# ZenGo-X/multi-party-ecdsa

Measured on AMD Instinct MI355X. Metric: GG20 signatures/sec (t=1, n=3; all parties of each session on the node's GPUs) + Paillier-2048 modexp/s per GPU, higher is better.
Workload: dtype u32 limbs (radix 2^29) / u64 accumulators

## Files before the change

### multi_party_ecdsa_amd/csrc/mpe_internal.h

```cpp
#pragma once
#include <hip/hip_runtime.h>
#include <stdint.h>
#include <new>
#include <utility>
#include <string>
#include <vector>

#include "../../include/mpecdsa_hip.h"
#include "mpe_kernels_heavy.h"
#include "mpe_sched.h"

struct mpe_ctx {
  int device = 0;
  int cus = 256;
  int fb_window_bits = 13;
  int window_bits = 0;
  bool ec_lane_groups = true;
  bool adaptive_lanes = true;
  bool use_pown = true;
  bool use_pair = true;
  bool use_multiexp = true;
  bool use_crt = true;
  bool use_fixed_base = true;
  bool use_sliding = true;
  int wide_div = 4;
  int device_share = 1;
  int xwide_div = 16;
  bool merge_xn = true;
  int use_prio = 1;
  int ladder_prio = 1;
  int use_crt_n = 1;
  int no_pdl_ahead = 0;
  int no_r1_dlog_first = 0;
  int no_r1_inversion_ahead = 0;
  int merge_r1_quarters = 1;
  bool merge_r1 = true;
  size_t fb_budget_bytes = 0;
  int modexp_waves_per_cu = 8;
  int fb_split = 0;
  int gg20_trace = 0;
  int sampler_max_attempts = 128;
  int no_primaries = 0;
  int no_elect = 0;
  int grid_mode = 2;
  void* tables[6] = {nullptr, nullptr, nullptr, nullptr, nullptr, nullptr};
  size_t tables_bytes[6] = {0, 0, 0, 0, 0, 0};
  hipStream_t aux[3] = {nullptr, nullptr, nullptr};
  hipEvent_t ev_fork[2] = {nullptr, nullptr}, ev_join[3] = {nullptr, nullptr, nullptr};
  hipEvent_t ev_ahead = nullptr;
  hipEvent_t ev_mid = nullptr;
  bool aux_ready = false;
  bool allow_par = true;
  int par_items = 32768;
  void* ws = nullptr;
  size_t ws_bytes = 0, ws_off = 0;
  int ws_hold = 0;
  size_t ws_top = 0;
  void* sess_buf = nullptr;
  size_t sess_bytes = 0;
  bool sess_in_use = false;
  void* slab_buf = nullptr;
  size_t slab_bytes = 0;
  mpe_launch_info last = {};
  mpe_encoding enc = {};
  bool prof_on = false;
  struct ProfEvt { hipEvent_t a, b; int kind, bits, exp_words, batch, exp2_words; int wave_trips; };
  std::vector<ProfEvt> prof;
  uint32_t* prof_ctr = nullptr;
  int prof_ctr_cap = 0;
};

struct mpe_modset {
  int bits = 0;
  int count = 0;
  int K = 0;
  void* blob = nullptr;
  uint32_t* n_limbs = nullptr;
  uint32_t* one_limbs = nullptr;
  uint32_t* r2_limbs = nullptr;
  uint32_t* r2h_limbs = nullptr;
  uint32_t* n0inv = nullptr;
  uint32_t* words = nullptr;
  uint32_t* one_words = nullptr;
};

struct mpe_pairset {
  int half_bits = 0;
  int count = 0;
  void* blob = nullptr;
  uint32_t *n_limbs = nullptr, *n0inv = nullptr, *one = nullptr, *r2 = nullptr, *tp = nullptr, *kc = nullptr;
  const uint32_t* mod_words = nullptr;
};

void mpe_set_error(const char* what, hipError_t e);
void mpe_set_error_msg(const char* what);

namespace mpe {

inline Rows rows(const uint32_t* p, int stride, const int32_t* idx = nullptr, int words = 0) {
  return Rows{p, idx, stride, words};
}
inline Rows no_rows() { return Rows{nullptr, nullptr, 0, 0}; }

int launch_modexp(mpe_ctx* ctx, const mpe_modset* ms, int batch, Rows mod_sel, Rows base_lo, Rows base_hi, Rows exps,
                  int exp_words, uint32_t* out, hipStream_t st);
int launch_modexp2(mpe_ctx* ctx, const mpe_modset* ms, int batch, Rows mod_sel, Rows base, Rows exps, int exp_words,
                   Rows base2, Rows exps2, int exp2_words, uint32_t* out, hipStream_t st);
int launch_modmul(mpe_ctx* ctx, const mpe_modset* ms, int batch, Rows mod_sel, Rows a, Rows b, uint32_t* out,
                  hipStream_t st);
int modset_create_dev(mpe_ctx* ctx, int bits, int count, const uint32_t* d_moduli, mpe_modset** out, hipStream_t st);

void ctx_copy_options(mpe_ctx* dst, const mpe_ctx* src);
void prof_begin(mpe_ctx* ctx, hipStream_t st, int kind, int bits, int exp_words, int batch, int exp2_words = 0);
void prof_end(mpe_ctx* ctx, hipStream_t st);
uint32_t* prof_counter(mpe_ctx* ctx, int wave_trips);

int pairset_create_2048(int count, const uint32_t* d_moduli, mpe_pairset** out, hipStream_t st);
int pairset_create_1024(int count, const uint32_t* d_moduli, mpe_pairset** out, hipStream_t st);
int pair_modexp_2048(mpe_ctx* ctx, const mpe_pairset* ps, int batch, Rows mod_sel, Rows base, Rows exps, int exp_words,
                     Rows base2, Rows exps2, int exp2_words, int half, uint32_t* out, hipStream_t st, int public_exp);
int pair_modexp_1024(mpe_ctx* ctx, const mpe_pairset* ps, int batch, Rows mod_sel, Rows base, Rows exps, int exp_words,
                     Rows base2, Rows exps2, int exp2_words, int half, uint32_t* out, hipStream_t st, int public_exp);

int ws_reserve(mpe_ctx* ctx, size_t bytes, hipStream_t st);
void* ws_alloc(mpe_ctx* ctx, size_t bytes);
uint32_t* tables_for(mpe_ctx* ctx, size_t need, hipStream_t st);
bool ensure_aux(mpe_ctx* ctx);

struct Fork {
  mpe_ctx* ctx; hipStream_t main; int n, first; bool on;
  Fork(mpe_ctx* c, hipStream_t m, int branches, bool enable, int first_aux = 0);
  hipStream_t s(int i) const { return (on && i > 0) ? ctx->aux[first + i - 1] : main; }
  void join();
  void branch_done_wait(int i, hipStream_t waiter);
};
struct WsTop {
  mpe_ctx* c;
  WsTop(mpe_ctx* ctx, const char* top) : c(ctx) { c->ws_top = (size_t)(((const char*)c->ws + c->ws_bytes) - top); }
  ~WsTop() { c->ws_top = 0; }
};
template <class T>
inline T* ws_array(mpe_ctx* ctx, size_t count) { return (T*)ws_alloc(ctx, count * sizeof(T)); }

inline int blocks_for(int n, int threads) { return (n + threads - 1) / threads; }

inline int persistent_grid(const mpe_ctx* ctx, int need, int cap);
inline int ladder_grid(const mpe_ctx* ctx, int units, int cap) {
  if (ctx->no_elect) return persistent_grid(ctx, units, cap);
  if (units <= cap) return (2 * units <= cap && !ctx->no_primaries) ? 2 * units : units;
  return cap;
}
inline SchedArgs ladder_sched(const mpe_ctx* ctx, int units, int cap, int32_t* state, hipStream_t st) {
  SchedArgs a{nullptr, SCHED_STATIC, units, ctx->use_prio ? ctx->ladder_prio : 0};
  if (ctx->no_elect || !state) return a;
  if (2 * units <= cap) { if (!ctx->no_primaries) { a.state = state; a.mode = SCHED_PRIMARIES; } }
  else if (units > cap) { a.state = state; a.mode = SCHED_ALL; }
  if (a.state) (void)hipMemsetAsync(a.state, 0, SCHED_WORDS * sizeof(int32_t), st);
  return a;
}
inline int persistent_grid(const mpe_ctx* ctx, int need, int cap) {
  if (need <= cap) return need;
  const int rem = need % cap;
  if (rem == 0) return cap;
  if (ctx->grid_mode == 1 || (ctx->grid_mode == 2 && 2 * rem <= cap)) return cap;
  const int trips = (need + cap - 1) / cap;
  return (need + trips - 1) / trips;
}

}
```

### multi_party_ecdsa_amd/csrc/mpe_lib.hip

```cpp
#include <string.h>
#include <initializer_list>
#include <mutex>
#include "mpe_internal.h"
#include "mpe_ec.h"

using namespace mpe;

thread_local std::string g_last_error;
void mpe_set_error(const char* what, hipError_t e) { g_last_error = std::string(what) + ": " + hipGetErrorString(e); }
void mpe_set_error_msg(const char* what) { g_last_error = what; }

namespace mpe {

int ws_reserve(mpe_ctx* ctx, size_t bytes, hipStream_t st) {
  if (ctx->ws_hold) {
    if (ctx->ws_off + bytes + ctx->ws_top > ctx->ws_bytes) { mpe_set_error_msg("workspace: the shared reservation is too small"); return MPE_E_NOMEM; }
    return MPE_OK;
  }
  ctx->ws_off = 0;
  if (bytes + ctx->ws_top <= ctx->ws_bytes) return MPE_OK;
  if (ctx->ws_top) { mpe_set_error_msg("workspace: cannot grow while a caller keeps arrays at its top"); return MPE_E_NOMEM; }
  if (ctx->ws) { (void)hipStreamSynchronize(st); (void)hipFree(ctx->ws); ctx->ws = nullptr; ctx->ws_bytes = 0; }
  const size_t want = bytes + (bytes >> 2) + (1u << 20);
  hipError_t e = hipMalloc(&ctx->ws, want);
// ... 1 lines not shown
  ctx->ws_bytes = want;
  return MPE_OK;
}
void* ws_alloc(mpe_ctx* ctx, size_t bytes) {
  const size_t off = (ctx->ws_off + 255) & ~(size_t)255;
  if (off + bytes + ctx->ws_top > ctx->ws_bytes) return nullptr;
  ctx->ws_off = off + bytes;
  return (char*)ctx->ws + off;
}

static int slot_of(const mpe_ctx* ctx, hipStream_t st) {
  for (int i = 0; i < 3; ++i) if (ctx->aux[i] && st == ctx->aux[i]) return i + 1;
  return 0;
}
uint32_t* tables_for(mpe_ctx* ctx, size_t need, hipStream_t st) {
  const int sl = slot_of(ctx, st);
  if (need > ctx->tables_bytes[sl]) {
    if (ctx->tables[sl]) { (void)hipStreamSynchronize(st); (void)hipFree(ctx->tables[sl]); ctx->tables[sl] = nullptr; ctx->tables_bytes[sl] = 0; }
    hipError_t e = hipMalloc(&ctx->tables[sl], need);
    if (e != hipSuccess) { mpe_set_error("hipMalloc(window tables)", e); return nullptr; }
    ctx->tables_bytes[sl] = need;
  }
  return (uint32_t*)ctx->tables[sl];
}
bool ensure_aux(mpe_ctx* ctx) {
  if (ctx->aux_ready) return true;
  for (int i = 0; i < 3; ++i) if (hipStreamCreateWithFlags(&ctx->aux[i], hipStreamNonBlocking) != hipSuccess) return false;
  for (int i = 0; i < 2; ++i) if (hipEventCreateWithFlags(&ctx->ev_fork[i], hipEventDisableTiming) != hipSuccess) return false;
  for (int i = 0; i < 3; ++i) if (hipEventCreateWithFlags(&ctx->ev_join[i], hipEventDisableTiming) != hipSuccess) return false;
  if (hipEventCreateWithFlags(&ctx->ev_mid, hipEventDisableTiming) != hipSuccess) return false;
  if (hipEventCreateWithFlags(&ctx->ev_ahead, hipEventDisableTiming) != hipSuccess) return false;
  ctx->aux_ready = true;
  return true;
}
Fork::Fork(mpe_ctx* c, hipStream_t m, int branches, bool enable, int first_aux) : ctx(c), main(m), n(branches), first(first_aux) {
  on = enable && c->allow_par && branches > 1 && first_aux + branches - 1 <= 3 && ensure_aux(c);
  if (!on) return;
  hipEvent_t ev = c->ev_fork[first_aux ? 1 : 0];
  (void)hipEventRecord(ev, m);
  for (int i = 1; i < n; ++i) (void)hipStreamWaitEvent(c->aux[first + i - 1], ev, 0);
}
void Fork::branch_done_wait(int i, hipStream_t waiter) {
  if (!on || i <= 0 || waiter == ctx->aux[first + i - 1]) return;
  (void)hipEventRecord(ctx->ev_join[first + i - 1], ctx->aux[first + i - 1]);
  (void)hipStreamWaitEvent(waiter, ctx->ev_join[first + i - 1], 0);
}
void Fork::join() {
  if (!on) return;
  for (int i = 1; i < n; ++i) {
    (void)hipEventRecord(ctx->ev_join[first + i - 1], ctx->aux[first + i - 1]);
    (void)hipStreamWaitEvent(main, ctx->ev_join[first + i - 1], 0);
  }
}

void prof_begin(mpe_ctx* ctx, hipStream_t st, int kind, int bits, int exp_words, int batch, int exp2_words) {
  if (!ctx->prof_on) return;
  mpe_ctx::ProfEvt ev;
  ev.kind = kind; ev.bits = bits; ev.exp_words = exp_words; ev.batch = batch; ev.exp2_words = exp2_words; ev.wave_trips = 0;
  (void)hipEventCreate(&ev.a);
  (void)hipEventCreate(&ev.b);
  (void)hipEventRecord(ev.a, st);
  ctx->prof.push_back(ev);
}
uint32_t* prof_counter(mpe_ctx* ctx, int wave_trips) {
  if (!ctx->prof_on || ctx->prof.empty() || !ctx->prof_ctr || (int)ctx->prof.size() > ctx->prof_ctr_cap) return nullptr;
  ctx->prof.back().wave_trips = wave_trips;
  return ctx->prof_ctr + (ctx->prof.size() - 1);
}
void prof_end(mpe_ctx* ctx, hipStream_t st) {
  if (ctx->prof_on && !ctx->prof.empty()) (void)hipEventRecord(ctx->prof.back().b, st);
}

static ModsetView view_of(const mpe_modset* ms) {
  ModsetView v;
  v.n_limbs = ms->n_limbs; v.one_limbs = ms->one_limbs; v.r2_limbs = ms->r2_limbs; v.r2h_limbs = ms->r2h_limbs;
  v.n0inv = ms->n0inv; v.count = ms->count;
  return v;
}

template <class C>
static int grid_for(const mpe_ctx* ctx, int batch, int waves_per_cu) {
  return persistent_grid(ctx, (batch + C::GROUPS - 1) / C::GROUPS, ctx->cus * waves_per_cu);
}

template <class C>
static int modset_create_impl(int count, const uint32_t* d_moduli, mpe_modset** out, hipStream_t st) {
  mpe_modset* ms = new (std::nothrow) mpe_modset();
  if (!ms) return MPE_E_NOMEM;
  ms->bits = C::BITS;
  ms->count = count;
  ms->K = C::K;
  const size_t words = (size_t)count * C::K;
  const size_t iw = (size_t)count * C::K32;
  const size_t total = (4 * words + (size_t)count + iw + 4) * sizeof(uint32_t);
  hipError_t e = hipMalloc(&ms->blob, total);
  if (e != hipSuccess) { delete ms; mpe_set_error("hipMalloc(modset)", e); return MPE_E_NOMEM; }
  uint32_t* p = (uint32_t*)ms->blob;
  ms->n_limbs = p;
  ms->one_limbs = p + words;
  ms->r2_limbs = p + 2 * words;
  ms->r2h_limbs = p + 3 * words;
  ms->n0inv = p + 4 * words;
  ms->words = ms->n0inv + count;
  ms->one_words = ms->words + iw;
  (void)hipMemcpyAsync(ms->words, d_moduli, iw * sizeof(uint32_t), hipMemcpyDeviceToDevice, st);
  (void)hipMemsetD32Async((hipDeviceptr_t)ms->one_words, 1, 1, st);
  const int blocks = (count + C::GROUPS - 1) / C::GROUPS;
  hipLaunchKernelGGL(modset_setup_kernel<C>, dim3(blocks), dim3(64), 0, st, count, d_moduli, ms->n_limbs,
                     ms->one_limbs, ms->r2_limbs, ms->r2h_limbs, ms->n0inv);
  e = hipGetLastError();
  if (e != hipSuccess) { (void)hipFree(ms->blob); delete ms; mpe_set_error("modset_setup_kernel", e); return MPE_E_HIP; }
  *out = ms;
  return MPE_OK;
}

int modset_create_dev(mpe_ctx* ctx, int bits, int count, const uint32_t* d_moduli, mpe_modset** out, hipStream_t st) {
  (void)ctx;
  if (bits == 4096) return modset_create_impl<Cfg4096>(count, d_moduli, out, st);
  if (bits == 2048) return modset_create_impl<Cfg2048>(count, d_moduli, out, st);
  return MPE_E_ARG;
}

template <class C>
static int modexp_impl(mpe_ctx* ctx, const mpe_modset* ms, int batch, Rows mod_sel, Rows base_lo, Rows base_hi, Rows exps,
                       int exp_words, Rows base2, Rows exps2, int exp2_words, uint32_t* d_out, hipStream_t st) {
  const int units = (batch + C::GROUPS - 1) / C::GROUPS, cap = ctx->cus * ctx->modexp_waves_per_cu;
  const int grid = ladder_grid(ctx, units, cap);
  int wb = exp_words <= 8 ? 4 : (exp_words < 48 ? 5 : 6);
  if (ctx->window_bits) wb = ctx->window_bits;
  const bool dual = base2.p != nullptr;
  if (dual && (base_hi.p != nullptr || exp2_words <= 0 || 32 * exp2_words > ((exp_words * 32 + wb - 1) / wb - 1) * wb)) {
    mpe_set_error_msg("modexp: the second exponent must be shorter than the first");
    return MPE_E_ARG;
  }
  const size_t need = (size_t)grid * C::GROUPS * (((size_t)1 << wb) + (dual ? 16 : 0)) * C::K * sizeof(uint32_t);
  uint32_t* tabs = tables_for(ctx, need + SCHED_WORDS * sizeof(int32_t), st);
  if (!tabs) return MPE_E_NOMEM;
  const SchedArgs sched = ladder_sched(ctx, units, cap, (int32_t*)((char*)tabs + need), st);
  prof_begin(ctx, st, 0, C::BITS, exp_words, batch, dual ? exp2_words : 0);
  hipLaunchKernelGGL(modexp_kernel<C>, dim3(grid), dim3(64), 0, st, batch, view_of(ms), mod_sel, base_lo, base_hi, exps,
                     exp_words, wb, base2, exps2, exp2_words, d_out, tabs, sched);
  prof_end(ctx, st);
  hipError_t e = hipGetLastError();
  if (e != hipSuccess) { mpe_set_error("modexp_kernel", e); return MPE_E_HIP; }
  ctx->last.waves = grid;
  ctx->last.ints_per_wave = C::GROUPS;
  ctx->last.limbs = C::K;
  ctx->last.limb_bits = C::W;
  ctx->last.lds_bytes_per_wave = C::LDS_WORDS * 4;
  ctx->last.table_scratch_bytes = need;
  return MPE_OK;
}

int launch_modexp2(mpe_ctx* ctx, const mpe_modset* ms, int batch, Rows mod_sel, Rows base, Rows exps, int exp_words,
                   Rows base2, Rows exps2, int exp2_words, uint32_t* out, hipStream_t st) {
  if (batch == 0) return MPE_OK;
  if (ms->bits == 4096)
    return modexp_impl<Cfg4096>(ctx, ms, batch, mod_sel, base, no_rows(), exps, exp_words, base2, exps2, exp2_words, out, st);
  if (ms->bits == 2048)
    return modexp_impl<Cfg2048>(ctx, ms, batch, mod_sel, base, no_rows(), exps, exp_words, base2, exps2, exp2_words, out, st);
  return MPE_E_ARG;
}
int launch_modexp(mpe_ctx* ctx, const mpe_modset* ms, int batch, Rows mod_sel, Rows base_lo, Rows base_hi, Rows exps,
                  int exp_words, uint32_t* out, hipStream_t st) {
  if (batch == 0) return MPE_OK;
  if (ms->bits == 4096)
    return modexp_impl<Cfg4096>(ctx, ms, batch, mod_sel, base_lo, base_hi, exps, exp_words, no_rows(), no_rows(), 0, out, st);
  if (ms->bits == 2048)
    return modexp_impl<Cfg2048>(ctx, ms, batch, mod_sel, base_lo, base_hi, exps, exp_words, no_rows(), no_rows(), 0, out, st);
  return MPE_E_ARG;
}

template <class C>
static int modmul_impl(mpe_ctx* ctx, const mpe_modset* ms, int batch, Rows mod_sel, Rows a, Rows b, uint32_t* d_out,
                       hipStream_t st) {
  const int grid = grid_for<C>(ctx, batch, 16);
  prof_begin(ctx, st, 1, C::BITS, 0, batch);
  hipLaunchKernelGGL(modmul_kernel<C>, dim3(grid), dim3(64), 0, st, batch, view_of(ms), mod_sel, a, b, d_out);
  prof_end(ctx, st);
  hipError_t e = hipGetLastError();
  if (e != hipSuccess) { mpe_set_error("modmul_kernel", e); return MPE_E_HIP; }
  return MPE_OK;
}

int launch_modmul(mpe_ctx* ctx, const mpe_modset* ms, int batch, Rows mod_sel, Rows a, Rows b, uint32_t* out,
                  hipStream_t st) {
  if (batch == 0) return MPE_OK;
  if (ms->bits == 4096) return modmul_impl<Cfg4096>(ctx, ms, batch, mod_sel, a, b, out, st);
  if (ms->bits == 2048) return modmul_impl<Cfg2048>(ctx, ms, batch, mod_sel, a, b, out, st);
  return MPE_E_ARG;
}

static Rows mod_selector(const mpe_modset* ms, const int32_t* d_mod_idx) {
  return Rows{nullptr, d_mod_idx, (d_mod_idx == nullptr && ms->count != 1) ? 1 : 0, 0};
}

}

#include "mpe_small.h"

namespace mpe {
static void pairset_free(mpe_pairset* ps) {
  if (!ps) return;
  if (ps->blob) (void)hipFree(ps->blob);
  delete ps;
}
static int pairset_create(int half_bits, int count, const uint32_t* d_moduli, mpe_pairset** out, hipStream_t st) {
  if (half_bits == 2048) return pairset_create_2048(count, d_moduli, out, st);
  if (half_bits == 1024) return pairset_create_1024(count, d_moduli, out, st);
  return MPE_E_ARG;
}
static int launch_pair_modexp(mpe_ctx* ctx, const mpe_pairset* ps, int batch, Rows mod_sel, Rows base, Rows exps, int exp_words,
                              Rows base2, Rows exps2, int exp2_words, uint32_t* out, hipStream_t st, int half = 0, int public_exp = 0) {
  if (batch == 0) return MPE_OK;
  if (ps->half_bits == 2048)
    return pair_modexp_2048(ctx, ps, batch, mod_sel, base, exps, exp_words, base2, exps2, exp2_words, half, out, st, public_exp);
  if (ps->half_bits == 1024)
    return pair_modexp_1024(ctx, ps, batch, mod_sel, base, exps, exp_words, base2, exps2, exp2_words, half, out, st, public_exp);
  return MPE_E_ARG;
}
}
#include "mpe_paillier.h"
#include "mpe_proofs.h"
#include "mpe_mta.h"
#include "mpe_bob.h"
#include "mpe_gg20.h"
#include "mpe_sample.h"
#include "mpe_pipeline.h"
#include "mpe_comm.h"
#include "mpe_sigma.h"
#include "mpe_blame.h"
#include "mpe_keygen.h"
#include "mpe_primes.h"
#include "mpe_lindell.h"

extern "C" {

const char* mpe_version(void) { return "mpecdsa-hip 0.7.0 (gfx950)"; }
const char* mpe_last_error(void) { return g_last_error.c_str(); }

void mpe_encoding_default(mpe_encoding* e) {
  if (!e) return;
  memset(e, 0, sizeof *e);
  e->ck_salt = 0x4B5A656Eu;
  for (int i = 0; i < 4; ++i) e->ord_dlog[i] = e->ord_cdlog[i] = (uint8_t)i;
  for (int i = 0; i < 8; ++i) e->ord_pedersen[i] = e->ord_heg[i] = e->ord_ecddh[i] = (uint8_t)i;
}
static bool is_perm(const uint8_t* o, int n) {
  unsigned seen = 0;
  for (int i = 0; i < n; ++i) { if (o[i] >= n || (seen >> o[i]) & 1u) return false; seen |= 1u << o[i]; }
  return true;
}
int mpe_ctx_set_encoding(mpe_ctx* ctx, const mpe_encoding* e) {
  if (!ctx || !e) return MPE_E_ARG;
  if (e->chain_point > 1 || e->zero_bytes > 1 || e->ck_mask_order > 1 || e->reserved != 0 || !is_perm(e->ord_dlog, 3) ||
      !is_perm(e->ord_pedersen, 5) || !is_perm(e->ord_heg, 7) || !is_perm(e->ord_ecddh, 6) || !is_perm(e->ord_cdlog, 4)) {
    mpe_set_error_msg("mpe_ctx_set_encoding: a flag is not 0/1 or an order is not a permutation");
    return MPE_E_ARG;
  }
  ctx->enc = *e;
  return MPE_OK;
}
int mpe_ctx_set_device_share(mpe_ctx* ctx, int contexts) {
  if (!ctx || contexts < 1 || contexts > 64) return MPE_E_ARG;
  ctx->device_share = contexts;
  return MPE_OK;
}
int mpe_ctx_get_encoding(const mpe_ctx* ctx, mpe_encoding* out) {
  if (!ctx || !out) return MPE_E_ARG;
  *out = ctx->enc;
  return MPE_OK;
}

namespace mpe {
struct CtxOption {
  const char* key;
  long lo, hi;
  void (*set)(mpe_ctx*, long);
  long (*get)(const mpe_ctx*);
};
#define MPE_OPT_BOOL_OFF(name, field) {name, 0, 1, [](mpe_ctx* c, long v) { c->field = !v; }, [](const mpe_ctx* c) -> long { return c->field ? 0 : 1; }}
#define MPE_OPT_INT(name, lo, hi, field) {name, lo, hi, [](mpe_ctx* c, long v) { c->field = (decltype(c->field))v; }, [](const mpe_ctx* c) -> long { return (long)c->field; }}
static const CtxOption kCtxOptions[] = {
    MPE_OPT_BOOL_OFF("no_fixed_base", use_fixed_base),
    MPE_OPT_BOOL_OFF("no_crt", use_crt),
    MPE_OPT_BOOL_OFF("no_multiexp", use_multiexp),
    MPE_OPT_BOOL_OFF("no_pair", use_pair),
    MPE_OPT_BOOL_OFF("no_pown", use_pown),
    MPE_OPT_BOOL_OFF("no_sliding", use_sliding),
    MPE_OPT_BOOL_OFF("no_par", allow_par),
    MPE_OPT_BOOL_OFF("no_wide", adaptive_lanes),
    MPE_OPT_BOOL_OFF("no_ec_lane_groups", ec_lane_groups),
    MPE_OPT_BOOL_OFF("no_merge_xn", merge_xn),
    MPE_OPT_BOOL_OFF("no_merge_r1", merge_r1),
    MPE_OPT_INT("fb_window_bits", 4, 16, fb_window_bits),
    MPE_OPT_INT("window_bits", 0, 6, window_bits),
    MPE_OPT_INT("wide_div", 1, 64, wide_div),
    MPE_OPT_INT("merge_r1_quarters", 0, 64, merge_r1_quarters),
    MPE_OPT_INT("no_r1_inversion_ahead", 0, 1, no_r1_inversion_ahead),
    MPE_OPT_BOOL_OFF("no_prio", use_prio),
    MPE_OPT_INT("no_pdl_ahead", 0, 1, no_pdl_ahead),
    MPE_OPT_BOOL_OFF("no_crt_n", use_crt_n),
    MPE_OPT_INT("no_r1_dlog_first", 0, 1, no_r1_dlog_first),
    MPE_OPT_INT("xwide_div", 0, 1 << 20, xwide_div),
    MPE_OPT_INT("waves_per_cu", 1, 8, modexp_waves_per_cu),
    MPE_OPT_INT("grid_mode", 0, 2, grid_mode),
    MPE_OPT_INT("fb_split", 0, 64, fb_split),
    MPE_OPT_INT("gg20_trace", 0, 1, gg20_trace),
    MPE_OPT_INT("sampler_max_attempts", 1, 1 << 20, sampler_max_attempts),
    MPE_OPT_INT("no_primaries", 0, 1, no_primaries),
    MPE_OPT_INT("no_elect", 0, 1, no_elect),
    {"fb_budget_mb", 0, 1 << 20, [](mpe_ctx* c, long v) { c->fb_budget_bytes = (size_t)v << 20; }, [](const mpe_ctx* c) -> long { return (long)(c->fb_budget_bytes >> 20); }},
};
#undef MPE_OPT_BOOL_OFF
#undef MPE_OPT_INT
extern "C++" void ctx_copy_options(mpe_ctx* dst, const mpe_ctx* src) {
  for (const CtxOption& o : kCtxOptions) o.set(dst, o.get(src));
}
}

int mpe_ctx_set_option(mpe_ctx* ctx, const char* key, const char* value) {
  if (!ctx || !key || !value) return MPE_E_ARG;
  if (!strcmp(key, "grid")) {
    const int m = !strcmp(value, "equal") ? 0 : (!strcmp(value, "full") ? 1 : (!strcmp(value, "hybrid") ? 2 : -1));
    if (m < 0) { mpe_set_error_msg("mpe_ctx_set_option: grid = equal | full | hybrid"); return MPE_E_ARG; }
    ctx->grid_mode = m;
    return MPE_OK;
  }
  if (!strcmp(key, "no_adaptive_lanes")) {
    const bool off = atoi(value) != 0;
    ctx->adaptive_lanes = !off; ctx->ec_lane_groups = !off;
    return MPE_OK;
  }
  for (const mpe::CtxOption& o : mpe::kCtxOptions) {
    if (strcmp(key, o.key)) continue;
    char* end = nullptr;
    const long v = strtol(value, &end, 10);
    if (end == value || *end || v < o.lo || v > o.hi) {
      mpe_set_error_msg((std::string("mpe_ctx_set_option: ") + key + " takes an integer in [" + std::to_string(o.lo) + ", " + std::to_string(o.hi) + "]").c_str());
      return MPE_E_ARG;
    }
    if (!strcmp(key, "window_bits") && v == 1) { mpe_set_error_msg("mpe_ctx_set_option: window_bits takes 0 (auto) or 2..6"); return MPE_E_ARG; }
    o.set(ctx, v);
    return MPE_OK;
  }
  mpe_set_error_msg((std::string("mpe_ctx_set_option: unknown option ") + key).c_str());
  return MPE_E_ARG;
}
int mpe_ctx_get_option(const mpe_ctx* ctx, const char* key, long* value) {
  if (!ctx || !key || !value) return MPE_E_ARG;
  for (const mpe::CtxOption& o : mpe::kCtxOptions)
    if (!strcmp(key, o.key)) { *value = o.get(ctx); return MPE_OK; }
  return MPE_E_ARG;
}
int mpe_ctx_option_count(void) { return (int)(sizeof(mpe::kCtxOptions) / sizeof(mpe::kCtxOptions[0])); }
const char* mpe_ctx_option_name(int i) { return (i >= 0 && i < mpe_ctx_option_count()) ? mpe::kCtxOptions[i].key : nullptr; }

int mpe_ctx_create(mpe_ctx** out, int device) {
  if (!out) return MPE_E_ARG;
  hipError_t e = hipSetDevice(device);
  if (e != hipSuccess) { mpe_set_error("hipSetDevice", e); return MPE_E_HIP; }
  hipDeviceProp_t prop;
  e = hipGetDeviceProperties(&prop, device);
  if (e != hipSuccess) { mpe_set_error("hipGetDeviceProperties", e); return MPE_E_HIP; }
  mpe_ctx* c = new (std::nothrow) mpe_ctx();
  if (!c) return MPE_E_NOMEM;
  c->device = device;
  c->cus = prop.multiProcessorCount;
  mpe_encoding_default(&c->enc);
  static std::once_flag comb_once[64];
  static hipError_t comb_err[64];
  if (device < 0 || device >= 64) { delete c; return MPE_E_ARG; }
  std::call_once(comb_once[device], [device]() {
    hipLaunchKernelGGL(mpe::ec::ec_comb_build_kernel, dim3(2), dim3(64), 0, 0);
    comb_err[device] = hipDeviceSynchronize();
  });
  e = comb_err[device];
  if (e != hipSuccess) { mpe_set_error("ec_comb_build_kernel", e); delete c; return MPE_E_HIP; }
  *out = c;
  return MPE_OK;
}

int mpe_ctx_wipe(mpe_ctx* ctx, void* stream) {
  if (!ctx) return MPE_E_ARG;
  hipStream_t st = (hipStream_t)stream;
  for (int i = 0; i < 6; ++i) if (ctx->tables[i]) (void)hipMemsetAsync(ctx->tables[i], 0, ctx->tables_bytes[i], st);
  if (ctx->ws) (void)hipMemsetAsync(ctx->ws, 0, ctx->ws_bytes, st);
  const hipError_t e = hipGetLastError();
  if (e != hipSuccess) { mpe_set_error("mpe_ctx_wipe", e); return MPE_E_HIP; }
  return MPE_OK;
}

__global__ void count_nonzero_kernel(const uint32_t* __restrict__ p, size_t words, unsigned long long* __restrict__ out) {
  size_t g = (size_t)blockIdx.x * blockDim.x + threadIdx.x;
  const size_t step = (size_t)gridDim.x * blockDim.x;
  unsigned long long c = 0;
  for (; g < words; g += step) c += p[g] != 0u;
  if (c) atomicAdd(out, c);
}
int mpe_ctx_scratch_audit(mpe_ctx* ctx, uint64_t* nonzero_words, uint64_t* total_bytes, void* stream) {
  if (!ctx || !nonzero_words) return MPE_E_ARG;
  hipStream_t st = (hipStream_t)stream;
  unsigned long long* d = nullptr;
  hipError_t e = hipMalloc((void**)&d, 8);
  if (e != hipSuccess) { mpe_set_error("hipMalloc(audit)", e); return MPE_E_NOMEM; }
  (void)hipMemsetAsync(d, 0, 8, st);
  const void* ptrs[11] = {ctx->tables[0], ctx->tables[1], ctx->tables[2], ctx->tables[3], ctx->tables[4], ctx->tables[5], ctx->ws,
                          nullptr, nullptr, ctx->sess_buf, ctx->slab_buf};
  const size_t bytes[11] = {ctx->tables_bytes[0], ctx->tables_bytes[1], ctx->tables_bytes[2], ctx->tables_bytes[3], ctx->tables_bytes[4],
                            ctx->tables_bytes[5], ctx->ws_bytes, 0, 0, ctx->sess_bytes, ctx->slab_bytes};
  uint64_t tot = 0;
  for (int i = 0; i < 11; ++i) {
    if (!ptrs[i] || !bytes[i]) continue;
    tot += bytes[i];
    hipLaunchKernelGGL(count_nonzero_kernel, dim3(4096), dim3(256), 0, st, (const uint32_t*)ptrs[i], bytes[i] / 4, d);
  }
  unsigned long long h = 0;
  e = hipMemcpyAsync(&h, d, 8, hipMemcpyDeviceToHost, st);
  if (e == hipSuccess) e = hipStreamSynchronize(st);
  (void)hipFree(d);
  if (e != hipSuccess) { mpe_set_error("mpe_ctx_scratch_audit", e); return MPE_E_HIP; }
  *nonzero_words = h;
  if (total_bytes) *total_bytes = tot;
  return MPE_OK;
}

int mpe_ctx_destroy(mpe_ctx* ctx) {
  if (!ctx) return MPE_E_ARG;
  (void)mpe_ctx_wipe(ctx, nullptr);
  if (ctx->sess_buf) { (void)hipMemsetAsync(ctx->sess_buf, 0, ctx->sess_bytes, nullptr); }
  if (ctx->slab_buf) { (void)hipMemsetAsync(ctx->slab_buf, 0, ctx->slab_bytes, nullptr); }
  (void)hipDeviceSynchronize();
  if (ctx->sess_buf) (void)hipFree(ctx->sess_buf);
  if (ctx->slab_buf) (void)hipFree(ctx->slab_buf);
  for (int i = 0; i < 6; ++i) if (ctx->tables[i]) (void)hipFree(ctx->tables[i]);
  if (ctx->ws) (void)hipFree(ctx->ws);
  if (ctx->aux_ready) {
    for (int i = 0; i < 3; ++i) { (void)hipStreamDestroy(ctx->aux[i]); (void)hipEventDestroy(ctx->ev_join[i]); }
    for (int i = 0; i < 2; ++i) (void)hipEventDestroy(ctx->ev_fork[i]);
    if (ctx->ev_mid) (void)hipEventDestroy(ctx->ev_mid);
    if (ctx->ev_ahead) (void)hipEventDestroy(ctx->ev_ahead);
  }
  for (auto& ev : ctx->prof) { (void)hipEventDestroy(ev.a); (void)hipEventDestroy(ev.b); }
  if (ctx->prof_ctr) (void)hipFree(ctx->prof_ctr);
  delete ctx;
  return MPE_OK;
}

int mpe_sync(mpe_ctx* ctx, void* stream) {
  (void)ctx;
  hipError_t e = hipStreamSynchronize((hipStream_t)stream);
  if (e != hipSuccess) { mpe_set_error("hipStreamSynchronize", e); return MPE_E_HIP; }
  return MPE_OK;
}

int mpe_last_launch_info(const mpe_ctx* ctx, mpe_launch_info* out) {
  if (!ctx || !out) return MPE_E_ARG;
  *out = ctx->last;
  return MPE_OK;
}

int mpe_prof_enable(mpe_ctx* ctx, int on) {
  if (!ctx) return MPE_E_ARG;
  for (auto& ev : ctx->prof) { (void)hipEventDestroy(ev.a); (void)hipEventDestroy(ev.b); }
  ctx->prof.clear();
  ctx->prof_on = on != 0;
  if (ctx->prof_on) {
    if (!ctx->prof_ctr) {
      ctx->prof_ctr_cap = 1 << 16;
      if (hipMalloc((void**)&ctx->prof_ctr, (size_t)ctx->prof_ctr_cap * sizeof(uint32_t)) != hipSuccess) { ctx->prof_ctr = nullptr; ctx->prof_ctr_cap = 0; }
    }
    if (ctx->prof_ctr) (void)hipMemset(ctx->prof_ctr, 0, (size_t)ctx->prof_ctr_cap * sizeof(uint32_t));
  }
  return MPE_OK;
}

int mpe_prof_collect(mpe_ctx* ctx, mpe_prof_rec* out, int max_records, int* n_out) {
  if (!ctx || !out || !n_out) return MPE_E_ARG;
  int n = 0;
  std::vector<uint32_t> ctr;
  size_t ix = 0;
  if (ctx->prof_ctr && !ctx->prof.empty()) (void)hipDeviceSynchronize();
  for (auto& ev : ctx->prof) {
    const size_t my = ix++;
    if (n >= max_records) break;
    if (hipEventSynchronize(ev.b) != hipSuccess) continue;
    float ms = 0.f;
    if (hipEventElapsedTime(&ms, ev.a, ev.b) != hipSuccess) continue;
    if (ctr.empty() && ctx->prof_ctr) {
      ctr.resize(ctx->prof.size() < (size_t)ctx->prof_ctr_cap ? ctx->prof.size() : (size_t)ctx->prof_ctr_cap);
      if (hipMemcpy(ctr.data(), ctx->prof_ctr, ctr.size() * sizeof(uint32_t), hipMemcpyDeviceToHost) != hipSuccess) ctr.assign(ctr.size(), 0u);
    }
    out[n].kind = ev.kind; out[n].bits = ev.bits; out[n].exp_words = ev.exp_words; out[n].batch = ev.batch; out[n].ms = ms;
    out[n].exp2_words = ev.exp2_words;
    out[n].sliding_frac = (ev.wave_trips > 0 && my < ctr.size()) ? (float)ctr[my] / (float)ev.wave_trips : (ev.kind == 6 ? -1.f : 0.f);
    ++n;
  }
  *n_out = n;
  return MPE_OK;
}

int mpe_modset_count(const mpe_modset* ms) { return ms ? ms->count : MPE_E_ARG; }
int mpe_modset_bits(const mpe_modset* ms) { return ms ? ms->bits : MPE_E_ARG; }

int mpe_modset_destroy(mpe_modset* ms) {
  if (!ms) return MPE_E_ARG;
  if (ms->blob) (void)hipFree(ms->blob);
  delete ms;
  return MPE_OK;
}

int mpe_modset_create(mpe_ctx* ctx, int bits, int count, const uint32_t* d_moduli, mpe_modset** out, void* stream) {
  if (!ctx || !out || !d_moduli || count <= 0) return MPE_E_ARG;
  return modset_create_dev(ctx, bits, count, d_moduli, out, (hipStream_t)stream);
}

int mpe_modexp(mpe_ctx* ctx, const mpe_modset* ms, int batch, const int32_t* d_mod_idx, const uint32_t* d_base,
               const uint32_t* d_exp, int exp_words, uint32_t* d_out, void* stream) {
  if (!ctx || !ms || !d_base || !d_exp || !d_out || batch < 0 || exp_words <= 0) return MPE_E_ARG;
  if (!d_mod_idx && ms->count != 1 && ms->count < batch) return MPE_E_ARG;
  const int k32 = ms->bits / 32;
  return launch_modexp(ctx, ms, batch, mod_selector(ms, d_mod_idx), rows(d_base, k32), no_rows(), rows(d_exp, exp_words),
                       exp_words, d_out, (hipStream_t)stream);
}

int mpe_modexp2(mpe_ctx* ctx, const mpe_modset* ms, int batch, const int32_t* d_mod_idx, const uint32_t* d_base,
                const uint32_t* d_exp, int exp_words, const uint32_t* d_base2, const uint32_t* d_exp2, int exp2_words,
                uint32_t* d_out, void* stream) {
  if (!ctx || !ms || !d_base || !d_exp || !d_base2 || !d_exp2 || !d_out || batch < 0 || exp_words <= 0 || exp2_words <= 0)
    return MPE_E_ARG;
  if (!d_mod_idx && ms->count != 1 && ms->count < batch) return MPE_E_ARG;
  const int k32 = ms->bits / 32;
  return launch_modexp2(ctx, ms, batch, mod_selector(ms, d_mod_idx), rows(d_base, k32), rows(d_exp, exp_words), exp_words,
                        rows(d_base2, k32), rows(d_exp2, exp2_words), exp2_words, d_out, (hipStream_t)stream);
}

int mpe_modmul(mpe_ctx* ctx, const mpe_modset* ms, int batch, const int32_t* d_mod_idx, const uint32_t* d_a,
               const uint32_t* d_b, uint32_t* d_out, void* stream) {
  if (!ctx || !ms || !d_a || !d_b || !d_out || batch < 0) return MPE_E_ARG;
  if (!d_mod_idx && ms->count != 1 && ms->count < batch) return MPE_E_ARG;
  const int k32 = ms->bits / 32;
  return launch_modmul(ctx, ms, batch, mod_selector(ms, d_mod_idx), rows(d_a, k32), rows(d_b, k32), d_out,
                       (hipStream_t)stream);
}

}
```

### multi_party_ecdsa_amd/csrc/mpe_pair1024.hip

```cpp
#include "mpe_pairexp.h"

namespace mpe {

int pairset_create_1024(int count, const uint32_t* d_moduli, mpe_pairset** out, hipStream_t st) {
  return pairset_create_impl<Cfg1024>(count, d_moduli, out, st);
}
int pair_modexp_1024(mpe_ctx* ctx, const mpe_pairset* ps, int batch, Rows mod_sel, Rows base, Rows exps, int exp_words,
                     Rows base2, Rows exps2, int exp2_words, int half, uint32_t* out, hipStream_t st, int public_exp) {
  using Wide = Cfg<1024, MPE_W, MPE_L / 2, 4>;
  static_assert(Wide::K == Cfg1024::K, "the two layouts share the limb arrays");
  const long resident = (long)ctx->cus * ctx->modexp_waves_per_cu * Cfg1024::GROUPS / ctx->device_share;
  using XWide = Cfg<1024, MPE_W, 5, 8>;
  const int xdiv = ctx->xwide_div;
  if (ctx->adaptive_lanes && xdiv > 0 && (long)xdiv * batch <= resident)
    return pair_modexp_impl<XWide>(ctx, ps, batch, mod_sel, base, exps, exp_words, base2, exps2, exp2_words, half, out, st, public_exp);
  if (ctx->adaptive_lanes && (long)ctx->wide_div * batch <= resident)
    return pair_modexp_impl<Wide>(ctx, ps, batch, mod_sel, base, exps, exp_words, base2, exps2, exp2_words, half, out, st, public_exp);
  return pair_modexp_impl<Cfg1024>(ctx, ps, batch, mod_sel, base, exps, exp_words, base2, exps2, exp2_words, half, out, st, public_exp);
}

}

#ifdef MPE_WAVE_TRACE
extern "C" int mpe_wave_trace_arm_1024(void* d_buf, unsigned cap) { return mpe::wave_trace_arm_impl(d_buf, cap); }
extern "C" int mpe_wave_trace_count_1024(unsigned* n) { return mpe::wave_trace_count_impl(n); }
#endif
```

### multi_party_ecdsa_amd/engine.py

```python
import ctypes as C
import os

import numpy as np
import torch

from . import _native as N
N_ = N
from .words import ints_to_words, words_to_ints


def _dev_u32(arr_np, device):
    return torch.from_numpy(arr_np.view(np.int32)).to(device)


def _to_np_u32(t):
    return t.detach().cpu().numpy().view(np.uint32)


_ENV_OPTIONS = ["no_fixed_base", "no_crt", "no_multiexp", "no_pair", "no_pown", "no_sliding", "no_par", "no_wide", "no_adaptive_lanes",
                "no_merge_xn", "no_merge_r1", "fb_window_bits", "window_bits", "wide_div", "xwide_div", "waves_per_cu", "grid", "fb_budget_mb",
                "fb_split", "gg20_trace", "sampler_max_attempts", "no_elect", "no_primaries", "merge_r1_quarters",
                "no_r1_inversion_ahead", "no_r1_dlog_first", "no_prio", "no_pdl_ahead", "no_crt_n"]


def options_from_env(env=None):
    env = os.environ if env is None else env
    out = {}
    for k in _ENV_OPTIONS:
        v = env.get("MPE_" + k.upper())
        if v is not None and v != "":
            out[k] = v
    if env.get("MPE_GRID_EQUAL"):
        out["grid"] = "equal"
    return out


class Context:
    def __init__(self, device=0, encoding=None, options=None):
        if not torch.cuda.is_available():
            raise N.MpeError("no GPU visible: the HIP path cannot run (there is no CPU fallback)")
        self.device = torch.device("cuda", device)
        h = C.c_void_p()
        N.check(N.lib.mpe_ctx_create(C.byref(h), device), "mpe_ctx_create")
        self.h = h
        if encoding is not None:
            self.set_encoding(encoding)
        self.options = {}
        for k, v in {**options_from_env(), **(options or {})}.items():
            self.set_option(k, v)

    def set_option(self, key, value):
        N.check(N.lib.mpe_ctx_set_option(self.h, str(key).encode(), str(int(value) if isinstance(value, bool) else value).encode()), f"mpe_ctx_set_option({key})")
        self.options[key] = value

    def get_option(self, key):
        v = C.c_long(0)
        N.check(N.lib.mpe_ctx_get_option(self.h, str(key).encode(), C.byref(v)), f"mpe_ctx_get_option({key})")
        return v.value

    def set_device_share(self, contexts):
        N.check(N.lib.mpe_ctx_set_device_share(self.h, int(contexts)), "mpe_ctx_set_device_share")

    def set_encoding(self, encoding):
        e = encoding if isinstance(encoding, N.Encoding) else N.Encoding.from_dict(dict(encoding))
        N.check(N.lib.mpe_ctx_set_encoding(self.h, C.byref(e)), "mpe_ctx_set_encoding")

    def encoding(self):
        e = N.Encoding()
        N.check(N.lib.mpe_ctx_get_encoding(self.h, C.byref(e)), "mpe_ctx_get_encoding")
        return e.as_dict()

    def stream(self):
        return C.c_void_p(torch.cuda.current_stream(self.device).cuda_stream)

    def sync(self):
        N.check(N.lib.mpe_sync(self.h, self.stream()), "mpe_sync")

    def launch_info(self):
        li = N.LaunchInfo()
        N.check(N.lib.mpe_last_launch_info(self.h, C.byref(li)), "mpe_last_launch_info")
        return {k: getattr(li, k) for k, _ in li._fields_}

    def prof_enable(self, on=True):
        N.check(N.lib.mpe_prof_enable(self.h, int(on)), "mpe_prof_enable")

    def prof_collect(self, max_records=4096):
        arr = (N.ProfRec * max_records)()
        n = C.c_int(0)
        N.check(N.lib.mpe_prof_collect(self.h, arr, max_records, C.byref(n)), "mpe_prof_collect")
        return [dict(kind=r.kind, bits=r.bits, exp_words=r.exp_words, batch=r.batch, ms=r.ms, exp2_words=r.exp2_words,
                     sliding_frac=r.sliding_frac) for r in arr[:n.value]]

    def wipe(self):
        N.check(N.lib.mpe_ctx_wipe(self.h, self.stream()), "mpe_ctx_wipe")

    def scratch_audit(self):
        nz, tot = C.c_uint64(0), C.c_uint64(0)
        N.check(N.lib.mpe_ctx_scratch_audit(self.h, C.byref(nz), C.byref(tot), self.stream()), "mpe_ctx_scratch_audit")
        return nz.value, tot.value

    def close(self):
        if self.h:
            N.lib.mpe_ctx_destroy(self.h)
            self.h = None

    def __del__(self):
        try:
            self.close()
        except Exception:
            pass


class ModSet:

    def __init__(self, ctx, bits, moduli):
        self.ctx, self.bits, self.k32 = ctx, bits, bits // 32
        if isinstance(moduli, torch.Tensor):
            self.d_moduli = moduli.contiguous()
        else:
            self.d_moduli = _dev_u32(ints_to_words(moduli, self.k32), ctx.device)
        self.count = self.d_moduli.shape[0]
        h = C.c_void_p()
        N.check(N.lib.mpe_modset_create(ctx.h, bits, self.count, C.c_void_p(self.d_moduli.data_ptr()),
                                        C.byref(h), ctx.stream()), "mpe_modset_create")
        self.h = h

    def close(self):
        if self.h:
            N.lib.mpe_modset_destroy(self.h)
            self.h = None

    def __del__(self):
        try:
            self.close()
        except Exception:
            pass


def modexp_device(ctx, ms, d_base, d_exp, d_out=None, d_mod_idx=None):
    B = d_base.shape[0]
    if d_out is None:
        d_out = torch.empty_like(d_base)
    idx_ptr = C.c_void_p(d_mod_idx.data_ptr()) if d_mod_idx is not None else None
    N.check(N.lib.mpe_modexp(ctx.h, ms.h, B, idx_ptr, C.c_void_p(d_base.data_ptr()),
                             C.c_void_p(d_exp.data_ptr()), d_exp.shape[1], C.c_void_p(d_out.data_ptr()),
                             ctx.stream()), "mpe_modexp")
    return d_out


def modmul_device(ctx, ms, d_a, d_b, d_out=None, d_mod_idx=None):
    B = d_a.shape[0]
    if d_out is None:
        d_out = torch.empty_like(d_a)
    idx_ptr = C.c_void_p(d_mod_idx.data_ptr()) if d_mod_idx is not None else None
    N.check(N.lib.mpe_modmul(ctx.h, ms.h, B, idx_ptr, C.c_void_p(d_a.data_ptr()), C.c_void_p(d_b.data_ptr()),
                             C.c_void_p(d_out.data_ptr()), ctx.stream()), "mpe_modmul")
    return d_out


def mod_pow2(ctx, ms, bases, exps, bases2, exps2, mod_idx=None, exp_bits=None, exp2_bits=None):
    ew = ((exp_bits or max(1, max(int(e).bit_length() for e in exps))) + 31) // 32
    ew2 = ((exp2_bits or max(1, max(int(e).bit_length() for e in exps2))) + 31) // 32
    dv = lambda xs, w: _dev_u32(ints_to_words(xs, w), ctx.device)
    d_idx = torch.tensor(mod_idx, dtype=torch.int32, device=ctx.device) if mod_idx is not None else None
    d_b, d_e, d_b2, d_e2 = dv(bases, ms.k32), dv(exps, ew), dv(bases2, ms.k32), dv(exps2, ew2)
    d_out = torch.empty_like(d_b)
    N.check(N.lib.mpe_modexp2(ctx.h, ms.h, len(bases), C.c_void_p(d_idx.data_ptr()) if d_idx is not None else None,
                              C.c_void_p(d_b.data_ptr()), C.c_void_p(d_e.data_ptr()), ew, C.c_void_p(d_b2.data_ptr()),
                              C.c_void_p(d_e2.data_ptr()), ew2, C.c_void_p(d_out.data_ptr()), ctx.stream()), "mpe_modexp2")
    ctx.sync()
    return words_to_ints(_to_np_u32(d_out))


def mod_pow(ctx, ms, bases, exps, mod_idx=None, exp_bits=None):
    if exp_bits is None:
        exp_bits = max(1, max(int(e).bit_length() for e in exps))
    ew = (exp_bits + 31) // 32
    d_base = _dev_u32(ints_to_words(bases, ms.k32), ctx.device)
    d_exp = _dev_u32(ints_to_words(exps, ew), ctx.device)
    d_idx = torch.tensor(mod_idx, dtype=torch.int32, device=ctx.device) if mod_idx is not None else None
    d_out = modexp_device(ctx, ms, d_base, d_exp, d_mod_idx=d_idx)
    ctx.sync()
    return words_to_ints(_to_np_u32(d_out))


def mod_mul(ctx, ms, a, b, mod_idx=None):
    d_a = _dev_u32(ints_to_words(a, ms.k32), ctx.device)
    d_b = _dev_u32(ints_to_words(b, ms.k32), ctx.device)
    d_idx = torch.tensor(mod_idx, dtype=torch.int32, device=ctx.device) if mod_idx is not None else None
    d_out = modmul_device(ctx, ms, d_a, d_b, d_mod_idx=d_idx)
    ctx.sync()
    return words_to_ints(_to_np_u32(d_out))


def _ptr(t):
    return C.c_void_p(t.data_ptr()) if t is not None else None


class PaillierKeys:

    def __init__(self, ctx, N=None, p=None, q=None):
        self.ctx = ctx
        h = C.c_void_p()
        if p is not None:
            self.d_p = p if torch.is_tensor(p) else _dev_u32(ints_to_words(p, 32), ctx.device)
            self.d_q = q if torch.is_tensor(q) else _dev_u32(ints_to_words(q, 32), ctx.device)
            N_.check(N_.lib.mpe_paillier_create_private(ctx.h, len(p), _ptr(self.d_p), _ptr(self.d_q), C.byref(h),
                                                        ctx.stream()), "mpe_paillier_create_private")
            self.private = True
        else:
            self.d_N = _dev_u32(ints_to_words(N, 64), ctx.device)
            N_.check(N_.lib.mpe_paillier_create_public(ctx.h, len(N), _ptr(self.d_N), C.byref(h), ctx.stream()),
                     "mpe_paillier_create_public")
            self.private = False
        self.h = h
        self.nkeys = N_.lib.mpe_paillier_nkeys(h)

    def close(self):
        if self.h:
            N_.lib.mpe_paillier_destroy(self.h)
            self.h = None

    def __del__(self):
        try:
            self.close()
        except Exception:
            pass

    def encrypt_device(self, d_m, d_r, d_key_idx=None, d_c=None):
        B = d_m.shape[0]
        if d_c is None:
            d_c = torch.empty((B, 128), dtype=torch.int32, device=d_m.device)
        N_.check(N_.lib.mpe_paillier_encrypt(self.ctx.h, self.h, B, _ptr(d_key_idx), _ptr(d_m), _ptr(d_r), _ptr(d_c),
                                             self.ctx.stream()), "mpe_paillier_encrypt")
        return d_c

    def decrypt_device(self, d_c, d_key_idx=None, d_m=None):
        B = d_c.shape[0]
        if d_m is None:
            d_m = torch.empty((B, 64), dtype=torch.int32, device=d_c.device)
        N_.check(N_.lib.mpe_paillier_decrypt(self.ctx.h, self.h, B, _ptr(d_key_idx), _ptr(d_c), _ptr(d_m),
                                             self.ctx.stream()), "mpe_paillier_decrypt")
        return d_m

    def add_device(self, d_c1, d_c2, d_key_idx=None):
        out = torch.empty_like(d_c1)
        N_.check(N_.lib.mpe_paillier_add(self.ctx.h, self.h, d_c1.shape[0], _ptr(d_key_idx), _ptr(d_c1), _ptr(d_c2),
                                         _ptr(out), self.ctx.stream()), "mpe_paillier_add")
        return out

    def mul_device(self, d_c, d_k, d_key_idx=None):
        out = torch.empty_like(d_c)
        N_.check(N_.lib.mpe_paillier_mul(self.ctx.h, self.h, d_c.shape[0], _ptr(d_key_idx), _ptr(d_c), _ptr(d_k),
                                         d_k.shape[1], _ptr(out), self.ctx.stream()), "mpe_paillier_mul")
        return out

    def _idx(self, key_idx):
        return None if key_idx is None else torch.tensor(key_idx, dtype=torch.int32, device=self.ctx.device)

    def encrypt(self, m, r, key_idx=None):
        d = self.encrypt_device(_dev_u32(ints_to_words(m, 64), self.ctx.device),
                                _dev_u32(ints_to_words(r, 64), self.ctx.device), self._idx(key_idx))
        self.ctx.sync()
        return words_to_ints(_to_np_u32(d))

    def decrypt(self, c, key_idx=None):
        d = self.decrypt_device(_dev_u32(ints_to_words(c, 128), self.ctx.device), self._idx(key_idx))
        self.ctx.sync()
        return words_to_ints(_to_np_u32(d))

    def add(self, c1, c2, key_idx=None):
        d = self.add_device(_dev_u32(ints_to_words(c1, 128), self.ctx.device),
                            _dev_u32(ints_to_words(c2, 128), self.ctx.device), self._idx(key_idx))
        self.ctx.sync()
        return words_to_ints(_to_np_u32(d))

    def mul(self, c, k, key_idx=None, k_words=8):
        d = self.mul_device(_dev_u32(ints_to_words(c, 128), self.ctx.device),
                            _dev_u32(ints_to_words(k, k_words), self.ctx.device), self._idx(key_idx))
        self.ctx.sync()
        return words_to_ints(_to_np_u32(d))


def _new(ctx, B, words):
    return torch.empty((B, words), dtype=torch.int32, device=ctx.device)


def _flags(ctx, B):
    return torch.empty((B,), dtype=torch.uint8, device=ctx.device)


def dev(ctx, vals, words):
    return _dev_u32(ints_to_words(vals, words), ctx.device)


def host(t):
    return words_to_ints(_to_np_u32(t))


def modinv_device(ctx, ms, d_a, d_mod_idx=None):
    B = d_a.shape[0]
    out, ok = torch.empty_like(d_a), _flags(ctx, B)
    N_.check(N_.lib.mpe_modinv(ctx.h, ms.h, B, _ptr(d_mod_idx), _ptr(d_a), _ptr(out), _ptr(ok), ctx.stream()), "mpe_modinv")
    return out, ok


def ec_mul_base(ctx, d_k):
    out = _new(ctx, d_k.shape[0], 16)
    N_.check(N_.lib.mpe_ec_mul_base(ctx.h, d_k.shape[0], _ptr(d_k), d_k.shape[1], _ptr(out), ctx.stream()), "mpe_ec_mul_base")
    return out


def ec_mul(ctx, d_k, d_P):
    out = _new(ctx, d_k.shape[0], 16)
    N_.check(N_.lib.mpe_ec_mul(ctx.h, d_k.shape[0], _ptr(d_k), d_k.shape[1], _ptr(d_P), _ptr(out), ctx.stream()), "mpe_ec_mul")
    return out


def ec_add(ctx, d_P, d_Q):
    out = _new(ctx, d_P.shape[0], 16)
    N_.check(N_.lib.mpe_ec_add(ctx.h, d_P.shape[0], _ptr(d_P), _ptr(d_Q), _ptr(out), ctx.stream()), "mpe_ec_add")
    return out


def dlog_prove(ctx, d_sk, d_nonce):
# ... 708 lines not shown
```

Baseline: 18660.

## Add lean single-half modexp kernel for 1024-bit pair half requests

Adds a dedicated kernel for the case where only one half of a 1024-bit CRT pair is requested. Instead of running the generic pair kernel with a half flag, it does one windowed modexp, with an optional dual second base and exponent, per group and zero-fills the upper output words. The aim is to drop the per-step cost of the generic two-modulus path and use a smaller table footprint. Lane-width selection is unchanged, and the new path can be turned off with an option.

```diff
diff --git a/multi_party_ecdsa_amd/csrc/mpe_halfexp.h b/multi_party_ecdsa_amd/csrc/mpe_halfexp.h
--- /dev/null
+++ b/multi_party_ecdsa_amd/csrc/mpe_halfexp.h
@@ -0,0 +1,193 @@
+#pragma once
+#include "mpe_pairexp.h"
+
+namespace mpe {
+
+template <class C>
+__device__ __forceinline__ void copy_half_row_to_lds(uint32_t* gl, const uint32_t* __restrict__ row, const Lane& ln) {
+  static_assert(C::K % 4 == 0 && C::STRIDE % 2 == 0, "a row is whole 16-byte chunks and the group regions are 8-byte aligned");
+  constexpr int CHUNKS = C::K / 4;
+  const uint4* __restrict__ r4 = reinterpret_cast<const uint4*>(row);
+  uint2* l2 = reinterpret_cast<uint2*>(gl);
+#pragma unroll
+  for (int i = 0; i < (CHUNKS + C::TPI - 1) / C::TPI; ++i) {
+    const int ch = ln.t + C::TPI * i;
+    if ((i + 1) * C::TPI <= CHUNKS || ch < CHUNKS) {
+      const uint4 v = r4[ch];
+      l2[2 * ch] = make_uint2(v.x, v.y);
+      l2[2 * ch + 1] = make_uint2(v.z, v.w);
+    }
+  }
+}
+
+template <class C>
+__global__ void __launch_bounds__(64) half_modexp_kernel(int batch, PairsetView ps, Rows mod_sel, Rows base, Rows exps, int exp_words, int wb,
+                                                         Rows base2, Rows exps2, int exp2_words, uint32_t* __restrict__ out,
+                                                         uint32_t* __restrict__ tables, SchedArgs sched) {
+  __shared__ __attribute__((aligned(16))) uint32_t lds[C::LDS_WORDS];
+  const Lane ln = make_lane<C>();
+  uint32_t* gl = lds + ln.g * C::STRIDE;
+  constexpr int K = C::K, KS = pair_kstore(C::BITS);
+  const int slot = blockIdx.x * C::GROUPS + ln.g;
+  const int nslots = gridDim.x * C::GROUPS;
+  const bool dual = base2.p != nullptr;
+  const int TE = 1 << wb;
+  uint32_t* tab = tables + (size_t)slot * (TE + (dual ? 16 : 0)) * K;
+  uint32_t* tab2 = tab + (size_t)TE * K;
+  const int nwin = (exp_words * 32 + wb - 1) / wb;
+  const int nwin2 = dual ? exp2_words * 8 : 0;
+  const int top_bit = (nwin - 1) * wb;
+  const int words1 = base.words ? base.words : 2 * C::K32, words2 = base2.words ? base2.words : 2 * C::K32;
+  WaveSched ws;
+  ws.init(sched);
+
+#pragma unroll 1
+  for (;;) {
+    int ubase;
+    if (!ws.next(sched, batch, nslots, C::GROUPS, ubase)) break;
+    const int inst = ubase + ln.g;
+    const bool active = inst < batch;
+    const int idx = active ? inst : batch - 1;
+    const int mi = sel_index(mod_sel, idx);
+    const uint32_t* ex = row_of(exps, idx);
+    const uint32_t* ex2 = dual ? row_of(exps2, idx) : ex;
+
+    uint32_t n[C::L];
+    load_owner<C>(n, ps.n_limbs + (size_t)mi * KS, ln);
+    const uint32_t n0inv = ps.n0inv[mi];
+    {
+      uint32_t t0[C::L];
+      load_owner<C>(t0, ps.one + (size_t)mi * 2 * KS, ln);
+      store_owner<C>(tab, t0, ln);
+    }
+
+    uint32_t cur[C::L];
+    int which = 0;
+    const uint32_t* bw = row_of(base, idx);
+    int kin = (words1 + C::K32 - 1) / C::K32 - 1;
+    load_words_as_limbs<C>(cur, gl, bw + kin * C::K32, words1 - kin * C::K32, ln);
+    int ph = kin > 0 ? PP_IN : PP_MONT;
+    --kin;
+    int k = 0, b = top_bit;
+#pragma unroll 1
+    while (ph != PP_DONE) {
+      if (ph == PP_IN) {
+        copy_to_lds<C>(gl, ps.tp + (size_t)mi * 2 * KS, ln);
+      } else if (ph == PP_MONT) {
+        copy_to_lds<C>(gl, ps.r2 + (size_t)mi * 2 * KS, ln);
+      } else if (ph == PP_TAB) {
+        if (k == 1) put_limbs<C>(gl, cur, ln);
+      } else if (ph == PP_SQ) {
+        put_limbs<C>(gl, cur, ln);
+      } else if (ph == PP_MUL1) {
+        const uint32_t w = exp_window(ex, exp_words, b / wb, wb);
+        copy_half_row_to_lds<C>(gl, tab + (size_t)w * K, ln);
+      } else if (ph == PP_MUL2) {
+        const int wi = b >> 2;
+        const uint32_t w = (ex2[wi >> 3] >> ((wi & 7) * 4)) & 15u;
+        copy_half_row_to_lds<C>(gl, w ? tab2 + (size_t)w * K : tab, ln);
+      } else {
+#pragma unroll
+        for (int i = 0; i < C::L; ++i) gl[ln.t * C::L + i] = (ln.t == 0 && i == 0) ? 1u : 0u;
+      }
+      wave_lds_sync();
+      {
+        uint32_t r[C::L];
+        uint64_t c[C::L];
+#pragma unroll
+        for (int i = 0; i < C::L; ++i) c[i] = 0;
+        cios1<C, false>(r, c, cur, gl, gl, n, n0inv, ln);
+        wave_lds_sync();
+#pragma unroll
+        for (int i = 0; i < C::L; ++i) cur[i] = r[i];
+      }
+
+      bool tables_done = false;
+      if (ph == PP_IN) {
+        uint32_t ch[C::L];
+        load_words_as_limbs<C>(ch, gl, bw + kin * C::K32, C::K32, ln);
+        int64_t z[C::L];
+#pragma unroll
+        for (int i = 0; i < C::L; ++i) z[i] = (int64_t)cur[i] + (int64_t)ch[i];
+        full_normalize<C>(z, ln);
+#pragma unroll
+        for (int i = 0; i < C::L; ++i) cur[i] = (uint32_t)z[i];
+        if (--kin < 0) ph = PP_MONT;
+      } else if (ph == PP_MONT) {
+        store_owner<C>((which ? tab2 : tab) + K, cur, ln);
+        k = 1;
+        ph = PP_TAB;
+      } else if (ph == PP_TAB) {
+        ++k;
+        store_owner<C>((which ? tab2 : tab) + (size_t)k * K, cur, ln);
+        if (k > (which ? 14 : TE - 2)) {
+          if (!which && dual) {
+            which = 1;
+            bw = row_of(base2, idx);
+            kin = (words2 + C::K32 - 1) / C::K32 - 1;
+            load_words_as_limbs<C>(cur, gl, bw + kin * C::K32, words2 - kin * C::K32, ln);
+            ph = kin > 0 ? PP_IN : PP_MONT;
+            --kin;
+          } else {
+            tables_done = true;
+          }
+        }
+      } else if (ph == PP_FINAL) {
+        ph = PP_DONE;
+      } else {
+        if (ph == PP_SQ) --b;
+        const bool m1 = ph == PP_SQ && (b % wb) == 0;
+        const bool m2 = ph != PP_MUL2 && dual && (b & 3) == 0 && (b >> 2) < nwin2;
+        ph = m1 ? PP_MUL1 : (m2 ? PP_MUL2 : (b == 0 ? PP_FINAL : PP_SQ));
+      }
+      if (tables_done) {
+        __builtin_amdgcn_fence(__ATOMIC_SEQ_CST, "workgroup");
+        const uint32_t w = exp_window(ex, exp_words, nwin - 1, wb);
+        load_owner<C>(cur, tab + (size_t)w * K, ln);
+        b = top_bit;
+        ph = b == 0 ? PP_FINAL : PP_SQ;
+      }
+    }
+    reduce_once<C>(cur, n, ln);
+    uint32_t* o = out + (size_t)idx * 2 * C::K32;
+    store_limbs_as_words<C>(o, gl, cur, active, ln);
+    if (active)
+      for (int q = ln.t; q < C::K32; q += C::TPI) o[C::K32 + q] = 0u;
+  }
+}
+
+template <class C>
+int half_modexp_impl(mpe_ctx* ctx, const mpe_pairset* ps, int batch, Rows mod_sel, Rows base, Rows exps, int exp_words,
+                     Rows base2, Rows exps2, int exp2_words, uint32_t* d_out, hipStream_t st) {
+  const int units = (batch + C::GROUPS - 1) / C::GROUPS;
+  const int cap = ctx->cus * ctx->modexp_waves_per_cu;
+  const int grid = ladder_grid(ctx, units, cap);
+  int wb = exp_words <= 8 ? 4 : (exp_words < 48 ? 5 : 6);
+  if (ctx->window_bits) wb = ctx->window_bits;
+  const bool dual = base2.p != nullptr;
+  if (dual && (exp2_words <= 0 || 32 * exp2_words > ((exp_words * 32 + wb - 1) / wb - 1) * wb)) {
+    mpe_set_error_msg("pair modexp: the second exponent must be shorter than the first");
+    return MPE_E_ARG;
+  }
+  const size_t need = (size_t)grid * C::GROUPS * (((size_t)1 << wb) + (dual ? 16 : 0)) * C::K * sizeof(uint32_t);
+  uint32_t* tabs = tables_for(ctx, need + SCHED_WORDS * sizeof(int32_t), st);
+  if (!tabs) return MPE_E_NOMEM;
+  SchedArgs sched = ladder_sched(ctx, units, cap, (int32_t*)((char*)tabs + need), st);
+  if (sched.prio == 1) sched.prio = 2;
+  PairsetView v{ps->n_limbs, ps->n0inv, ps->one, ps->r2, ps->tp, ps->kc, ps->count};
+  prof_begin(ctx, st, 4, C::BITS, exp_words, batch, dual ? exp2_words : 0);
+  hipLaunchKernelGGL(half_modexp_kernel<C>, dim3(grid), dim3(64), 0, st, batch, v, mod_sel, base, exps, exp_words, wb, base2, exps2,
+                     exp2_words, d_out, tabs, sched);
+  prof_end(ctx, st);
+  hipError_t e = hipGetLastError();
+  if (e != hipSuccess) { mpe_set_error("half_modexp_kernel", e); return MPE_E_HIP; }
+  ctx->last.waves = grid;
+  ctx->last.ints_per_wave = C::GROUPS;
+  ctx->last.limbs = C::K;
+  ctx->last.limb_bits = C::W;
+  ctx->last.lds_bytes_per_wave = C::LDS_WORDS * 4;
+  ctx->last.table_scratch_bytes = need;
+  return MPE_OK;
+}
+
+}
diff --git a/multi_party_ecdsa_amd/csrc/mpe_internal.h b/multi_party_ecdsa_amd/csrc/mpe_internal.h
--- a/multi_party_ecdsa_amd/csrc/mpe_internal.h
+++ b/multi_party_ecdsa_amd/csrc/mpe_internal.h
@@ -30,6 +30,7 @@
   int use_prio = 1;
   int ladder_prio = 1;
   int use_crt_n = 1;
+  bool use_lean_half = true;
   int no_pdl_ahead = 0;
   int no_r1_dlog_first = 0;
   int no_r1_inversion_ahead = 0;
diff --git a/multi_party_ecdsa_amd/csrc/mpe_lib.hip b/multi_party_ecdsa_amd/csrc/mpe_lib.hip
--- a/multi_party_ecdsa_amd/csrc/mpe_lib.hip
+++ b/multi_party_ecdsa_amd/csrc/mpe_lib.hip
@@ -327,6 +327,7 @@
     MPE_OPT_INT("no_pdl_ahead", 0, 1, no_pdl_ahead),
     MPE_OPT_BOOL_OFF("no_crt_n", use_crt_n),
     MPE_OPT_INT("no_r1_dlog_first", 0, 1, no_r1_dlog_first),
+    MPE_OPT_BOOL_OFF("no_lean_half", use_lean_half),
     MPE_OPT_INT("xwide_div", 0, 1 << 20, xwide_div),
     MPE_OPT_INT("waves_per_cu", 1, 8, modexp_waves_per_cu),
     MPE_OPT_INT("grid_mode", 0, 2, grid_mode),
diff --git a/multi_party_ecdsa_amd/csrc/mpe_pair1024.hip b/multi_party_ecdsa_amd/csrc/mpe_pair1024.hip
--- a/multi_party_ecdsa_amd/csrc/mpe_pair1024.hip
+++ b/multi_party_ecdsa_amd/csrc/mpe_pair1024.hip
@@ -1,4 +1,5 @@
 #include "mpe_pairexp.h"
+#include "mpe_halfexp.h"
 
 namespace mpe {
 
@@ -12,6 +13,13 @@
   const long resident = (long)ctx->cus * ctx->modexp_waves_per_cu * Cfg1024::GROUPS / ctx->device_share;
   using XWide = Cfg<1024, MPE_W, 5, 8>;
   const int xdiv = ctx->xwide_div;
+  if (half && ctx->use_lean_half) {
+    if (ctx->adaptive_lanes && xdiv > 0 && (long)xdiv * batch <= resident)
+      return half_modexp_impl<XWide>(ctx, ps, batch, mod_sel, base, exps, exp_words, base2, exps2, exp2_words, out, st);
+    if (ctx->adaptive_lanes && (long)ctx->wide_div * batch <= resident)
+      return half_modexp_impl<Wide>(ctx, ps, batch, mod_sel, base, exps, exp_words, base2, exps2, exp2_words, out, st);
+    return half_modexp_impl<Cfg1024>(ctx, ps, batch, mod_sel, base, exps, exp_words, base2, exps2, exp2_words, out, st);
+  }
   if (ctx->adaptive_lanes && xdiv > 0 && (long)xdiv * batch <= resident)
     return pair_modexp_impl<XWide>(ctx, ps, batch, mod_sel, base, exps, exp_words, base2, exps2, exp2_words, half, out, st, public_exp);
   if (ctx->adaptive_lanes && (long)ctx->wide_div * batch <= resident)
diff --git a/multi_party_ecdsa_amd/engine.py b/multi_party_ecdsa_amd/engine.py
--- a/multi_party_ecdsa_amd/engine.py
+++ b/multi_party_ecdsa_amd/engine.py
@@ -20,7 +20,7 @@
 _ENV_OPTIONS = ["no_fixed_base", "no_crt", "no_multiexp", "no_pair", "no_pown", "no_sliding", "no_par", "no_wide", "no_adaptive_lanes",
                 "no_merge_xn", "no_merge_r1", "fb_window_bits", "window_bits", "wide_div", "xwide_div", "waves_per_cu", "grid", "fb_budget_mb",
                 "fb_split", "gg20_trace", "sampler_max_attempts", "no_elect", "no_primaries", "merge_r1_quarters",
-                "no_r1_inversion_ahead", "no_r1_dlog_first", "no_prio", "no_pdl_ahead", "no_crt_n"]
+                "no_r1_inversion_ahead", "no_r1_dlog_first", "no_prio", "no_pdl_ahead", "no_crt_n", "no_lean_half"]
 
 
 def options_from_env(env=None):
```

Result: no change. 18790 (median of 6 runs) (+0.7%).
